# zengyf131/gswt_renderer

Measured on AMD Instinct MI355X. Metric: frames/sec @1920x1080, 32x32 Wang-tile grid, higher is better.
Workload: dtype f32

## Files before the change

gswt_renderer_amd/_lib.py:

```python
from __future__ import annotations

import ctypes as C
import os

_HERE = os.path.dirname(os.path.abspath(__file__))
LIB_PATH = os.environ.get("GSWT_HIP_LIB") or os.path.join(_HERE, "lib", "libgswt_hip.so")

GSWT_OK = 0
GSWT_ERR_BAD_ARG = -1
GSWT_ERR_CAPACITY = -2
GSWT_ERR_HIP = -3
GSWT_ERR_STATE = -4
GSWT_ERR_RCCL = -6
GSWT_COMM_ID_BYTES = 128
GSWT_ORDER_REFERENCE = 0
GSWT_ORDER_DEPTH = 1
GSWT_OPT_NO_LOD_PREFILTER = 1
GSWT_OPT_DEBUG_VARYINGS = 2
GSWT_OPT_SEGMENT = 3
GSWT_DEFAULT_SEGMENT = 1536
GSWT_OPT_DEBUG_FLAGS = 4
GSWT_OPT_TIMING = 5
GSWT_OPT_PAIR_CAP = 6
GSWT_OPT_NO_MERGE_REUSE = 7
GSWT_OPT_DEFER_SWAP = 8
GSWT_OPT_GRAPH = 9
GSWT_OPT_STRICT_VS = 10
GSWT_OPT_DEPTH_PASSES = 12
GSWT_OPT_COMPOSITE = 13
GSWT_OPT_DEPTH_SORT = 14
GSWT_OPT_NO_CHUNK_CULL = 15
GSWT_OPT_ITEM_ORDER = 16
GSWT_SCENE_TEX = 0
GSWT_SCENE_RAW_DEPTH = 1
GSWT_SCENE_RAW_TABLES = 2
GSWT_SCENE_STATIC_LIST = 3
GSWT_SCENE_STATIC_BOXES = 4
GSWT_SCENE_LISTS = 5
GSWT_SCENE_BOUNDS = 6
GSWT_SHARD_ROWS = 0
GSWT_SHARD_COLUMNS = 1
GSWT_OUT_RGBA32F = 0
GSWT_OUT_RGBA8_UNORM = 1
GSWT_OUT_BGRA8_UNORM = 2
GSWT_VIDEO_NV12 = 16
GSWT_VIDEO_I420 = 17
GSWT_PROXY_SRC_RGBA8 = 0
GSWT_PROXY_SRC_RGBA16 = 1


class CameraUniforms(C.Structure):
    _fields_ = [("projection", C.c_float * 16), ("view", C.c_float * 16), ("focal", C.c_float * 2),
                ("viewport", C.c_float * 2), ("htan_fov", C.c_float * 4), ("cam_pos", C.c_float * 4)]


class SceneUniforms(C.Structure):
    _fields_ = [("splat_scale", C.c_float), ("tile_width", C.c_float), ("use_clip", C.c_uint32),
                ("clip_height", C.c_float), ("surface_type", C.c_uint32), ("sphere_radius", C.c_float),
                ("point_cloud_radius", C.c_float), ("transition_width_ratio", C.c_float),
                ("num_lod", C.c_uint32), ("draw_mode", C.c_uint32), ("map_half_wh", C.c_uint32 * 2),
                ("center_coord", C.c_int32 * 2), ("_pad0", C.c_uint32 * 2),
                ("transition_dist_vec", C.c_float * 16), ("height_map_scale", C.c_float * 4),
                ("scene_scale", C.c_float * 4)]


class TileUniforms(C.Structure):
    _fields_ = [("single_draw", C.c_uint32), ("map_index", C.c_uint32), ("single_lod_id", C.c_int32),
                ("valid_lod_id", C.c_int32), ("changing", C.c_uint32), ("changing_to_lower", C.c_int32),
                ("_pad0", C.c_uint32 * 2), ("tile_id", C.c_uint32 * 4), ("offset", C.c_float * 4),
                ("map_coord", C.c_uint32 * 4)]


# ... 179 lines not shown
```

gswt_renderer_amd/csrc/gswt_api.hip:

```cpp
#include "../../include/gswt_hip.h"
#include "gswt_device.h"

#include <dlfcn.h>

#include <algorithm>
#include <cstdarg>
#include <cstdio>
#include <cstring>
#include <string>
#include <unordered_map>
#include <utility>
#include <vector>

using namespace gswt;

namespace {

template <typename T>
struct DevBuf {
    T* p = nullptr;
    size_t cap = 0;
    DevBuf() = default;
    DevBuf(DevBuf&& o) noexcept : p(std::exchange(o.p, nullptr)), cap(std::exchange(o.cap, 0)) {}
    DevBuf& operator=(DevBuf&& o) noexcept { std::swap(p, o.p); std::swap(cap, o.cap); return *this; }
// ... 774 lines not shown
    c->static_n = arena_n; c->boxes_n = boxes_n;
    c->raw_cnt.assign(counts, counts + n_lt);
    c->raw_merge_offset = moff;
    c->raw_off.assign(n_lt * nv, 0);
    for (size_t i = 0; i < n_lt; i++) for (size_t v = 0; v < nv; v++) c->raw_off[i * nv + v] = (uint32_t)(nv * moff[i] + v * counts[i]);
    c->n_lod = n_lod; c->n_tile = n_tile; c->n_view = n_view;
    c->scene_ready = true;
    return GSWT_OK;
} GSWT_CATCH("gswt_upload_scene_rows")

int gswt_debug_read_scene(gswt_ctx* c, int what, void* out, size_t cap_bytes, size_t* n_bytes)
try {
    if (!c || !n_bytes) return GSWT_ERR_BAD_ARG;
    if (!c->scene_ready) return fail(c, GSWT_ERR_STATE, "gswt_debug_read_scene before a scene upload");
    const void* dev = nullptr;
    const void* hostp = nullptr;
    size_t bytes = 0;
    std::vector<uint32_t> tmp;
    switch (what) {
    case GSWT_SCENE_TEX: dev = c->tex.p; bytes = c->n_splats * 32; break;
    case GSWT_SCENE_RAW_DEPTH: {
        size_t total = 0;
        for (uint32_t k : c->raw_cnt) total += (size_t)k * c->n_view;
        dev = c->raw_depth.p; bytes = total * 4; break;
    }
    case GSWT_SCENE_RAW_TABLES:
        tmp = c->raw_off;
        tmp.insert(tmp.end(), c->raw_cnt.begin(), c->raw_cnt.end());
        tmp.insert(tmp.end(), c->raw_merge_offset.begin(), c->raw_merge_offset.end());
        hostp = tmp.data(); bytes = tmp.size() * 4; break;
    case GSWT_SCENE_STATIC_LIST: dev = c->static_list.p; bytes = c->static_n * 4; break;
    case GSWT_SCENE_STATIC_BOXES: dev = c->static_boxes.p; bytes = c->boxes_n * 24; break;
    case GSWT_SCENE_LISTS: hostp = c->lists.data(); bytes = c->lists.size() * sizeof(ListRef); break;
    case GSWT_SCENE_BOUNDS: {
        tmp.resize(7);
        memcpy(tmp.data(), c->loc_lo, 12); memcpy(tmp.data() + 3, c->loc_hi, 12); memcpy(tmp.data() + 6, &c->loc_max_trace, 4);
        hostp = tmp.data(); bytes = 28; break;
    }
    default: return fail(c, GSWT_ERR_BAD_ARG, "gswt_debug_read_scene: unknown item %d", what);
    }
    *n_bytes = bytes;
    if (!out) return GSWT_OK;
    if (cap_bytes < bytes) return fail(c, GSWT_ERR_CAPACITY, "gswt_debug_read_scene: buffer holds %zu bytes, need %zu", cap_bytes, bytes);
    if (hostp) { memcpy(out, hostp, bytes); return GSWT_OK; }
    hipSetDevice(c->device);
    HIP_TRY(c, sync_all(c));
    if (bytes) HIP_TRY(c, hipMemcpy(out, dev, bytes, hipMemcpyDeviceToHost));
    return GSWT_OK;
} GSWT_CATCH("gswt_debug_read_scene")

int gswt_configure(gswt_ctx* c, const float* height_map, int hm_w, int hm_h)
try {
    if (!c) return GSWT_ERR_BAD_ARG;
    hipSetDevice(c->device);
    HIP_TRY(c, collect_pending(c));
    if (!height_map || hm_w <= 0 || hm_h <= 0) { c->hm_w = c->hm_h = 0; return GSWT_OK; }
    HIP_TRY(c, c->hmap.ensure((size_t)hm_w * hm_h + 2));
    HIP_TRY(c, hipMemcpy(c->hmap.p, height_map, (size_t)hm_w * hm_h * 4, hipMemcpyHostToDevice));
    HIP_TRY(c, hipMemset(c->hmap.p + (size_t)hm_w * hm_h, 0, 8));
    {
        float mn = height_map[0], mx = height_map[0], du = 0.f, dv = 0.f;
        bool finite = true;
        for (int y = 0; y < hm_h; y++)
            for (int x = 0; x < hm_w; x++) {
                const float h = height_map[(size_t)y * hm_w + x];
                const float hr = height_map[(size_t)y * hm_w + (x + 1 == hm_w ? 0 : x + 1)], hd = height_map[(size_t)(y + 1 == hm_h ? 0 : y + 1) * hm_w + x];
// ... 309 lines not shown
        total += len;
    }
    if (total >= 0xFFFFFFFFull) return fail(c, GSWT_ERR_CAPACITY, "gswt_set_draws_merge_groups: merged lists exceed 2^32 entries");
    for (int i = 0; i < n_draws; i++)
        if (draws[i].merged) {
            const uint32_t g = draws[i].merged_group;
            if ((int)g >= n_groups || draws[i].merged_offset != desc[g].base || draws[i].merged_count != desc[g].len)
                return fail(c, GSWT_ERR_BAD_ARG, "gswt_set_draws_merge_groups: draw %d does not match group %u (offset %u/%u count %u/%u)", i, g,
                            draws[i].merged_offset, (int)g < n_groups ? desc[g].base : 0u, draws[i].merged_count, (int)g < n_groups ? desc[g].len : 0u);
        }
    int rc = set_draws_impl(c, draws, n_draws, nullptr, nullptr, nullptr, (size_t)total, true);
    if (rc != GSWT_OK) return rc;
    MergeSources msrc;
    for (int k = 0; k < kMergeSources; k++) { msrc.list[k] = nullptr; msrc.map[k] = nullptr; }
    D.src_mask = 0;
    for (int k : sources) {
        if (!c->sets[k].g_valid) return fail(c, GSWT_ERR_STATE, "gswt_set_draws_merge_groups: a source set lost its lists");
        msrc.list[k] = c->sets[k].merged_list.p; msrc.map[k] = c->sets[k].merged_map.p;
    }
    for (size_t q = 0; q < n_jobs; q++) D.src_mask |= 1u << jobs[q].src_set;
    D.g_desc.swap(desc);
    D.g_members.assign(members, members + n_members);
    D.g_valid = false;
    c->stat_groups_built += n_build; c->stat_groups_reused += n_jobs;
    hipStream_t s = c->set_stream;
    uint2* const h_cblocks = D.hp<uint2>(D.off_cblocks);
    uint2* const h_blocks = D.hp<uint2>(D.off_blocks);
    size_t n_cb = 0, n_blocks = 0;
    for (size_t q = 0; q < n_jobs; q++)
        for (uint32_t off = 0; off < jobs[q].len; off += 1024u) h_cblocks[n_cb++] = make_uint2((uint32_t)q, off);
    for (size_t q = 0; q < n_segs; q++)
        for (uint32_t off = 0; off < segs[q].len; off += 1024u) h_blocks[n_blocks++] = make_uint2((uint32_t)q, off);
    const uint32_t n_total = (uint32_t)build_total;
    memset(D.hp<uint8_t>(D.off_n64), 0, 64);
    *D.hp<unsigned long long>(D.off_n64) = n_total;
    HIP_TRY(c, hipMemcpyAsync(D.d_blob.p, D.h_blob.p, D.blob_bytes, hipMemcpyHostToDevice, s));
    launch_chunk_tabs(s, D.draws.p, D.xcd_first.p, D.n_draws, D.chunk_tab.p, D.chunk_tab_xcd.p, D.per_xcd, D.longest);
    if (n_jobs)
        launch_merge_copy(s, D.dp<MergeCopy>(D.off_jobs), D.dp<uint2>(D.off_cblocks), (uint32_t)n_cb, D.dp<uint2>(D.off_remap), msrc,
                          D.merged_list.p, D.merged_map.p);
    if (n_build) {
        int gbits = 1;
        while ((1u << gbits) < n_build) gbits++;
        const size_t radix_words = radix_ws_words(n_total, 16 + gbits);
        HIP_TRY(c, c->mg_ws.ensure_roomy(4 * (size_t)n_total + radix_words + 16));
        uint32_t* w = c->mg_ws.p;
        uint32_t* radix = w + 4 * (size_t)n_total;
        HIP_TRY(c, hipMemsetAsync(radix, 0, (radix_words + 16) * 4, s));
        launch_merge_build(s, D.dp<MergeSeg>(D.off_segs), (uint32_t)n_segs, D.dp<uint2>(D.off_blocks), (uint32_t)n_blocks, D.dp<MergeGroup>(D.off_groups),
                           (uint32_t)n_build, c->raw_depth.p, n_total, D.dp<unsigned long long>(D.off_n64), w, w + n_total, w + 2 * (size_t)n_total,
                           w + 3 * (size_t)n_total, radix, gbits, D.merged_list.p, D.merged_map.p);
    }
    HIP_TRY(c, hipGetLastError());
    HIP_TRY(c, hipEventRecord(D.ev_up, s));
    D.ev_up_pending = true; D.built = false;
    D.g_valid = true;
    publish_set(c, target);
    c->draws_ready = true;
    return GSWT_OK;
} GSWT_CATCH("gswt_set_draws_merge_groups")

int gswt_debug_read_merged(gswt_ctx* c, uint32_t* packed_list, uint32_t* map_id, size_t capacity, size_t* n)
try {
    if (!c || !n) return GSWT_ERR_BAD_ARG;
    const DrawSet& D = c->sets[c->cur_set];
    *n = D.n_merged;
    if (!packed_list || !map_id) return GSWT_OK;
    if (capacity < D.n_merged) return fail(c, GSWT_ERR_CAPACITY, "buffer holds %zu entries, need %zu", capacity, D.n_merged);
    hipSetDevice(c->device);
    HIP_TRY(c, sync_all(c));
    if (D.n_merged) {
        HIP_TRY(c, hipMemcpy(packed_list, D.merged_list.p, D.n_merged * 4, hipMemcpyDeviceToHost));
        HIP_TRY(c, hipMemcpy(map_id, D.merged_map.p, D.n_merged * 4, hipMemcpyDeviceToHost));
    }
    return GSWT_OK;
} GSWT_CATCH("gswt_debug_read_merged")

int gswt_shard_rows_padded(int height, int shard_count)
try {
    int tiles_y = (height + kTile - 1) / kTile;
    int sc = shard_count <= 1 ? 1 : shard_count;
// ... 1079 lines not shown
```

gswt_renderer_amd/csrc/gswt_device.h:

```cpp
#pragma once
#include <hip/hip_runtime.h>
#include <hip/hip_ext.h>
#include <hip/hip_fp16.h>
#include <stdint.h>
#include <string.h>
#include <type_traits>

namespace gswt {

constexpr int kTile = 16;
constexpr int kChunk = 256;
constexpr uint32_t kLodShift = 28;
constexpr uint32_t kIdxMask = (1u << kLodShift) - 1u;
constexpr int kOutF32 = 0, kOutRGBA8 = 1, kOutBGRA8 = 2;
constexpr int kOutNV12 = 16, kOutI420 = 17;
constexpr bool out_is_video(int out_format) { return out_format == kOutNV12 || out_format == kOutI420; }
inline size_t out_image_bytes(int out_format, int rows, int out_w)
{
    if (rows < 0 || out_w < 0) return 0;
    const size_t px = (size_t)rows * (size_t)out_w;
    if (out_format == kOutF32) return px * 16u;
    if (out_format == kOutRGBA8 || out_format == kOutBGRA8) return px * 4u;
    if (out_is_video(out_format)) return ((rows | out_w) & 1) ? 0 : px + px / 2u;
    return 0;
// ... 222 lines not shown
    uint2* partials_pick;
    hipEvent_t ev_pick_begin, ev_pick_end;
    uint32_t n_zero_head, n_zero_ranges, n_zero_depth;
};

void launch_chunk_tabs(hipStream_t s, const DrawDev* draws, const uint32_t* xcd_first, uint32_t n_draws, uint2* chunk_tab, uint2* chunk_tab_xcd,
                       const uint64_t per_xcd[8], uint64_t longest);
void launch_merge_build(hipStream_t s, const MergeSeg* segs, uint32_t n_segs, const uint2* blocks, uint32_t n_blocks, MergeGroup* groups, uint32_t n_groups,
                        const int32_t* raw, uint32_t n_total, const unsigned long long* n_total_dev, uint32_t* ka, uint32_t* va,
                        uint32_t* kb, uint32_t* vb, uint32_t* radix_ws, int group_bits, uint32_t* merged_list, uint32_t* merged_map);
int launch_scene_sort(hipStream_t s, const MergeSeg* segs, const uint2* blocks, uint32_t n_blocks, MergeGroup* groups, const int32_t* raw,
                      uint32_t n_total, const unsigned long long* n_total_dev, uint32_t* ka, uint32_t* va, uint32_t* kb, uint32_t* vb,
                      uint32_t* radix_ws, int group_bits);
void launch_scene_tex(hipStream_t s, const uint4* rows, uint32_t n, uint4* tex, int32_t* bounds);
void launch_scene_raw(hipStream_t s, const uint4* rows, uint32_t n, const uint32_t* moff, const uint32_t* cnt, uint32_t n_lt, const SceneViews& vps,
                      int32_t* raw);
void launch_scene_scatter(hipStream_t s, const MergeSeg* segs, uint32_t n_segs, const MergeGroup* groups, const uint32_t* sorted_keys,
                          const uint32_t* sorted_vals, uint32_t n_total, uint32_t* arena, uint32_t arena_n);
void launch_scene_self(hipStream_t s, const SceneList* lists, uint32_t n_lists, uint32_t lists_per_lod, uint32_t* arena);
void launch_scene_boxes(hipStream_t s, const SceneList* lists, uint32_t n_lists, uint32_t n_boxes, const uint32_t* arena, const uint4* tex,
                        uint32_t n_splats, float* boxes);
void launch_merge_copy(hipStream_t s, const MergeCopy* jobs, const uint2* blocks, uint32_t n_blocks, const uint2* remap, const MergeSources& src,
                       uint32_t* new_list, uint32_t* new_map);

void launch_cull(hipStream_t s, const Frame& f, const FrameBufs& b, bool chunk_cull);
void launch_project(hipStream_t s, const Frame& f, const FrameBufs& b, uint32_t n_launch, bool debug, bool strict);
void launch_emit(hipStream_t s, const Frame& f, const FrameBufs& b, uint32_t* keys, uint32_t* dkeys, uint32_t* krange, uint32_t n_launch);
void launch_composite(hipStream_t s, const Frame& f, const FrameBufs& b, const uint32_t* vals, int out_rows, int variant, const uint32_t* krange,
                      uint32_t depth_passes, bool report_max, bool heavy_first, hipEvent_t ev_begin, hipEvent_t ev_end, int out_format);
void launch_totals(hipStream_t s, uint32_t* super_sums, uint32_t n_super, unsigned long long* counters, uint32_t pair_cap);

size_t radix_ws_words(uint32_t n_cap, int key_bits);
size_t radix_ws_zero_words(uint32_t n_cap, int key_bits);
int launch_sort(hipStream_t s, uint32_t* keys_a, uint32_t* vals_a, uint32_t* keys_b, uint32_t* vals_b, uint32_t n_cap,
                const unsigned long long* n_ptr, int key_bits, uint32_t* ws, uint2* ranges = nullptr, const uint32_t* krange = nullptr,
                uint32_t* aux_a = nullptr, uint32_t* aux_b = nullptr);

void launch_tile_depth_sort(hipStream_t s, const uint2* ranges, uint32_t* vals, uint32_t* dkeys, uint32_t* vals_scratch, uint32_t* dkeys_scratch, int n_tiles,
                            uint32_t* long_list, unsigned long long* counters);
inline size_t tile_depth_list_words(size_t n_tiles) { return n_tiles + 1; }
uint32_t tile_depth_sort_cap();

void launch_unshard(hipStream_t s, const void* gathered, void* out, int width, int height, int shard_count, int rows_padded, int band_px,
                    int out_format);
void launch_skybox(hipStream_t s, const float* view16, float p00, float p11, int width, int height, int face_size, int equirect,
                   const float4* faces, float4* out);
void launch_skybox_bake(hipStream_t s, const SkyBakeArgs& a, const float4* equi, float4* faces);
void launch_proxy(hipStream_t s, const ProxyArgs& a, const float* hm, const float4* tex, float4* rgba, float* depth);
void launch_proxy_mip(hipStream_t s, const ProxyMipArgs& a, const uint8_t* src, int2* ranges, float* wv, float* wh, float4* tmp,
                      float4* part, float4* dst);
void launch_fill_f32(hipStream_t s, float* p, size_t n, float v);

}
```

gswt_renderer_amd/csrc/gswt_kernels.hip:

```cpp
#include "gswt_device.h"

namespace gswt {

__device__ __forceinline__ unsigned long long ballot64(bool p) { return __builtin_amdgcn_ballot_w64(p); }
__device__ __forceinline__ uint32_t lanes_below(unsigned long long m)
{
    return __builtin_amdgcn_mbcnt_hi((uint32_t)(m >> 32), __builtin_amdgcn_mbcnt_lo((uint32_t)m, 0u));
}

template <int CTRL, int ROW_MASK>
__device__ __forceinline__ uint32_t dpp_or_zero(uint32_t x)
{
    return (uint32_t)__builtin_amdgcn_update_dpp(0, (int)x, CTRL, ROW_MASK, 0xF, true);
}
__device__ __forceinline__ uint32_t wave_incl_scan(uint32_t v, uint32_t lane)
{
    (void)lane;
    v += dpp_or_zero<0x111, 0xF>(v);
    v += dpp_or_zero<0x112, 0xF>(v);
    v += dpp_or_zero<0x114, 0xF>(v);
    v += dpp_or_zero<0x118, 0xF>(v);
    v += dpp_or_zero<0x142, 0xA>(v);
    v += dpp_or_zero<0x143, 0xC>(v);
    return v;
// ... 164 lines not shown
        if (f.draw_mode == 3u) L = d.single_lod_id >= 0 ? (uint32_t)d.single_lod_id : lod_id;
        float cx = 0.0f, cy = 1.0f;
        if (L < 3u) cx = (3.0f - (float)L) / 3.0f;
        else cy = (6.0f - (float)L) / 3.0f;
        cr = 0.5f; cg = cx; cb = cy;
    } else if (f.draw_mode == 4u) {
        const uint32_t v = d.tile_view;
        float cx = 0.0f, cy = 0.0f;
        if (v < 4u) cx = (4.0f - (float)v) / 4.0f;
        if (v >= 4u) cy = (8.0f - (float)v) / 4.0f;
        if (v >= 8u) { cx = 1.0f; cy = 1.0f; }
        cr = 0.5f; cg = cx; cb = cy;
    }
}

__device__ __forceinline__ void tile_xy(const Frame& f, uint32_t tile, int& tx, int& ty)
{
    uint32_t q;
    if (f.tiles_x_magic != 0u && tile < 65536u) q = __umulhi(tile, f.tiles_x_magic);
    else q = tile / (uint32_t)f.tiles_x;
    tx = (int)(tile - q * (uint32_t)f.tiles_x); ty = (int)q;
}

__device__ __forceinline__ int owned_rows(int ty0, int ty1, int index, int count)
{
    if (count <= 1) return ty1 - ty0 + 1;
    int first = ty0 + ((index - ty0 % count) + count) % count;
    if (first > ty1) return 0;
    return (ty1 - first) / count + 1;
}

struct XcdLens { uint32_t len[8]; uint32_t longest; };
__global__ __launch_bounds__(256) void k_chunk_tabs(const DrawDev* __restrict__ draws, const uint32_t* __restrict__ xcd_first, uint32_t n_draws,
                                                    uint2* __restrict__ chunk_tab, uint2* __restrict__ chunk_tab_xcd, const XcdLens xl)
{
    const uint32_t d = blockIdx.x;
    if (d >= n_draws) {
        const uint32_t x = d - n_draws;
        for (uint32_t k = xl.len[x & 7u] + threadIdx.x; k < xl.longest; k += 256u) chunk_tab_xcd[(size_t)k * 8u + x] = make_uint2(0xFFFFFFFFu, 0xFFFFFFFFu);
        return;
    }
    const uint32_t nch = (draws[d].count + (uint32_t)kChunk - 1u) / (uint32_t)kChunk;
    const uint32_t c0 = draws[d].slot_base / (uint32_t)kChunk, x0 = xcd_first[d];
    for (uint32_t k = threadIdx.x; k < nch; k += 256u) {
        const uint2 e = make_uint2(d, k * (uint32_t)kChunk);
        chunk_tab[c0 + k] = e;
        chunk_tab_xcd[(size_t)(x0 + k) * 8u + (draws[d].xcd & 7u)] = e;
    }
}

__device__ __forceinline__ bool sphere_cell_box(const Frame& f, float bidx, float bidy, const float lo[3], const float hi[3], float blo[3], float bhi[3])
{
    const float xmax = ((float)f.map_half_wh[0] * 2.0f) * f.tile_width;
    const float block_w = xmax / 5.0f;
    const float ox = (float)(f.center_coord[0] - (int32_t)f.map_half_wh[0]) * f.tile_width + bidx * block_w;
    const float oy = (float)(f.center_coord[1] - (int32_t)f.map_half_wh[1]) * f.tile_width + bidy * block_w;
    const float bx0 = lo[0] - ox, bx1 = hi[0] - ox, by0 = lo[1] - oy, by1 = hi[1] - oy;
    if (!(block_w > 0.0f && bx0 >= 0.0f && bx1 <= block_w && by0 >= 0.0f && by1 <= block_w)) return false;
    constexpr int n = 3;
    const float R = fabsf(f.sphere_radius);
    const float zmax = fmaxf(fabsf(lo[2]), fabsf(hi[2]));
    const float rho = (R * 2.5f * ((bx1 - bx0) + (by1 - by0)) / (2.0f * (float)n * block_w) + zmax) * 1.02f + 1e-4f * R;
    if (!(rho == rho)) return false;
    for (int k = 0; k < 3; k++) { blo[k] = 3.402823466e+38f; bhi[k] = -3.402823466e+38f; }
    for (int j = 0; j < n; j++)
        for (int i = 0; i < n; i++) {
            float p[3];
            sphere_point(block_w, bidx, bidy, bx0 + (bx1 - bx0) * (((float)i + 0.5f) / (float)n), by0 + (by1 - by0) * (((float)j + 0.5f) / (float)n), p);
            for (int k = 0; k < 3; k++) { blo[k] = fminf(blo[k], p[k] * f.sphere_radius - rho); bhi[k] = fmaxf(bhi[k], p[k] * f.sphere_radius + rho); }
        }
    return blo[0] == blo[0] && bhi[0] == bhi[0] && blo[1] == blo[1] && bhi[1] == bhi[1] && blo[2] == blo[2] && bhi[2] == bhi[2];
}

__device__ __forceinline__ bool band_misses(const Frame& f, const float lo[3], const float hi[3], float bidx, float bidy)
{
    float blo[3], bhi[3];
    for (int k = 0; k < 3; k++) {
        const float a = lo[k] * f.scene_scale[k], b = hi[k] * f.scene_scale[k];
        blo[k] = fminf(a, b); bhi[k] = fmaxf(a, b);
    }
    if (f.surface_type == 1u) {
// ... 1004 lines not shown
        }
    }
    __syncthreads();
    GSWT_TR(4, GSWT_NOW())
    const uint32_t n_blk = min((uint32_t)kSortBlock, n - blk0);
#pragma unroll
    for (int k = 0; k < kSortItems; k++) {
        const uint32_t i = (uint32_t)k * kSortThreads + threadIdx.x;
        if (i < n_blk) {
            const uint2 kv = s_kv[i];
            const uint32_t gp = s_g[((kv.x - kmin) >> shift) & mask] + i;
            vals_out[gp] = kv.y;
            if (AUX == 2) aux_out[gp] = s_aux[AUX == 2 ? i : 0u];
            if (AUX == 1) aux_out[gp] = aux_in[blk0 + s_src[AUX == 1 ? i : 0u]];
            if (!ranges) keys_out[gp] = kv.x;
            else {
                const uint32_t kp = s_kv[i == 0u ? 0u : i - 1u].x, kn = s_kv[min(i + 1u, n_blk - 1u)].x;
                if (i == 0u || kp != kv.x) atomicMax(&ranges[kv.x].x, ~gp);
                if (i == n_blk - 1u || kn != kv.x) atomicMax(&ranges[kv.x].y, gp + 1u);
            }
        }
    }
    GSWT_TR(5, GSWT_NOW())
}

__device__ __forceinline__ uint32_t mg_find_seg(const MergeSeg* __restrict__ segs, uint32_t n_segs, uint32_t e)
{
    uint32_t lo = 0, hi = n_segs;
    while (hi - lo > 1u) { const uint32_t mid = (lo + hi) >> 1; if (segs[mid].start <= e) lo = mid; else hi = mid; }
    return lo;
}

__global__ __launch_bounds__(256) void k_mg_minmax(const MergeSeg* __restrict__ segs, const uint2* __restrict__ blocks, const int32_t* __restrict__ raw,
                                                   MergeGroup* __restrict__ groups)
{
    __shared__ int32_t s_mn[4], s_mx[4];
    const uint2 b = blocks[blockIdx.x];
    const MergeSeg sg = segs[b.x];
    int32_t mn = 2147483647, mx = -2147483647 - 1;
#pragma unroll
    for (uint32_t k = 0; k < 4u; k++) {
        const uint32_t i = b.y + k * 256u + threadIdx.x;
        const int32_t d = raw[sg.src + min(i, sg.len - 1u)];
        mn = min(mn, d); mx = max(mx, d);
    }
    for (int off = 32; off > 0; off >>= 1) { mn = min(mn, __shfl_down(mn, off, 64)); mx = max(mx, __shfl_down(mx, off, 64)); }
    if ((threadIdx.x & 63u) == 0) { s_mn[threadIdx.x >> 6] = mn; s_mx[threadIdx.x >> 6] = mx; }
    __syncthreads();
    if (threadIdx.x == 0) {
        atomicMin(&groups[sg.group].mn, min(min(s_mn[0], s_mn[1]), min(s_mn[2], s_mn[3])));
        atomicMax(&groups[sg.group].mx, max(max(s_mx[0], s_mx[1]), max(s_mx[2], s_mx[3])));
    }
}

__global__ __launch_bounds__(256) void k_mg_keys(const MergeSeg* __restrict__ segs, const uint2* __restrict__ blocks, const int32_t* __restrict__ raw,
                                                 const MergeGroup* __restrict__ groups, uint32_t* __restrict__ keys, uint32_t* __restrict__ vals)
{
    const uint2 b = blocks[blockIdx.x];
    const MergeSeg sg = segs[b.x];
    const MergeGroup g = groups[sg.group];
    const float depth_inv = 65535.0f / (float)(int32_t)((uint32_t)g.mx - (uint32_t)g.mn);
#pragma unroll
    for (uint32_t k = 0; k < 4u; k++) {
        const uint32_t i = b.y + k * 256u + threadIdx.x;
        if (i >= sg.len) break;
        const int32_t d = raw[sg.src + i];
        const float v = floorf((float)(int32_t)((uint32_t)d - (uint32_t)g.mn) * depth_inv);
        int32_t bk;
        if (v != v) bk = 0;
// ... 1000 lines not shown
        const int shard = x / band_px;
        src = ((size_t)shard * height + y) * band_px + (x - shard * band_px);
    } else {
        int ty = y >> 4;
        int shard = ty % shard_count, tyl = ty / shard_count;
        src = ((size_t)shard * rows_padded + (size_t)tyl * kTile + (y & 15)) * width + x;
    }
    out[(size_t)y * width + x] = gathered[src];
}

template <typename P, int TILE>
__global__ void k_unshard_plane(const P* __restrict__ gathered, P* __restrict__ out, int width, int height,
                                int shard_count, int rows_padded, int band_px, size_t stride)
{
    const int x = blockIdx.x * blockDim.x + threadIdx.x;
    const int y = blockIdx.y;
    if (x >= width || y >= height) return;
    size_t src;
    if (band_px > 0) {
        const int shard = x / band_px;
        src = (size_t)shard * stride + (size_t)y * band_px + (x - shard * band_px);
    } else {
        const int ty = y / TILE;
        const int shard = ty % shard_count, tyl = ty / shard_count;
        src = (size_t)shard * stride + ((size_t)tyl * TILE + (y % TILE)) * width + x;
    }
    out[(size_t)y * width + x] = gathered[src];
}

void launch_chunk_tabs(hipStream_t s, const DrawDev* draws, const uint32_t* xcd_first, uint32_t n_draws, uint2* chunk_tab, uint2* chunk_tab_xcd,
                       const uint64_t per_xcd[8], uint64_t longest)
{
    XcdLens xl;
    for (int x = 0; x < 8; x++) xl.len[x] = (uint32_t)per_xcd[x];
    xl.longest = (uint32_t)longest;
    if (n_draws) hipLaunchKernelGGL(k_chunk_tabs, dim3(n_draws + 8u), dim3(256), 0, s, draws, xcd_first, n_draws, chunk_tab, chunk_tab_xcd, xl);
}

GraphRec*& graph_recorder()
{
    static thread_local GraphRec* rec = nullptr;
    return rec;
}

bool kernel_events_enabled()
{
    static const bool on = !(getenv("GSWT_KERNEL_EVENTS") && atoi(getenv("GSWT_KERNEL_EVENTS")) == 0);
    return on;
}

void launch_cull(hipStream_t s, const Frame& f, const FrameBufs& b, bool chunk_cull)
{
    uint32_t grid = (b.n_chunks + 255u) / 256u;
    if (grid < 32) grid = 32;
    GSWT_LAUNCH(k_cull, dim3(grid), dim3(256), s, f, b.draws, b.draw_culled, b.cell_culled, b.n_cells, reinterpret_cast<uint32_t*>(b.counters), b.n_zero_head,
                reinterpret_cast<uint32_t*>(b.ranges), b.n_zero_ranges, b.block_sums, b.n_chunks, b.radix_depth, b.n_zero_depth,
                b.chunk_tab, b.n_chunks, b.boxes, chunk_cull && b.boxes ? 1u : 0u, b.live_cnt, b.live_tab, b.live_cid);
}

void launch_project(hipStream_t s, const Frame& f, const FrameBufs& b, uint32_t n_launch, bool debug, bool strict)
{
    if (b.n_chunks == 0) return;
    const uint32_t n_super = b.n_chunks / 256u + 1u;
    const bool full = f.surface_type == 2u || f.draw_mode != 0u;
#define GSWT_LAUNCH_PROJECT_S(D, F, S)                                                                                         \
    GSWT_LAUNCH((k_project<D, F, S>), dim3(n_launch), dim3(256), s, f, b.draws, b.chunk_tab_xcd, b.static_list, b.merged_list,   \
                b.merged_map, b.tex, b.hmap, b.draw_culled, b.cell_culled, b.live_cnt, b.live_tab, b.rects, b.recs, b.depths, b.block_sums, \
                b.super_sums, n_super, b.dbg, b.col_f)
#define GSWT_LAUNCH_PROJECT(D, F) do { if (strict) GSWT_LAUNCH_PROJECT_S(D, F, true); else GSWT_LAUNCH_PROJECT_S(D, F, false); } while (0)
// ... 7 lines not shown
}

void launch_emit(hipStream_t s, const Frame& f, const FrameBufs& b, uint32_t* keys, uint32_t* dkeys, uint32_t* krange, uint32_t n_launch)
{
    const uint32_t n_chunks = b.n_chunks, pair_cap = b.pair_cap;
    if (n_chunks == 0) return;
    const uint32_t n_super = n_chunks / 256u + 1u;
    const uint32_t* const excl = b.super_sums + 2u * kSuperStride * n_super;
    const float* const no_f = nullptr; uint32_t* const no_u = nullptr;
    const uint32_t* const cnt2 = n_launch ? b.live_cnt + 8u * kSuperStride : nullptr;
    const uint32_t* const cid = n_launch ? b.live_cid : nullptr;
    const dim3 grid(n_launch ? ((n_launch / 8u + kEmitGroup - 1u) / kEmitGroup) * 8u : (n_chunks + kEmitGroup - 1u) / kEmitGroup);
#define GSWT_LAUNCH_EMIT(D, L)                                                                                                 \
    GSWT_LAUNCH((k_emit<D, L>), grid, dim3(256), s, f, b.rects, b.block_sums, excl, n_chunks, pair_cap, b.counters, keys, b.vals_a, \
                D ? b.depths : no_f, D ? dkeys : no_u, D ? krange : no_u, cnt2, cid)
    if (n_launch) { if (dkeys) GSWT_LAUNCH_EMIT(true, true); else GSWT_LAUNCH_EMIT(false, true); }
    else if (dkeys) GSWT_LAUNCH_EMIT(true, false);
    else GSWT_LAUNCH_EMIT(false, false);
#undef GSWT_LAUNCH_EMIT
}

size_t radix_ws_words(uint32_t n_cap, int key_bits)
{
    const uint32_t nblk = (n_cap + kSortBlock - 1) / kSortBlock, nsup = (nblk >> kSupShift) + 1;
    const int passes = (key_bits + 7) / 8;
    return (size_t)passes * ((size_t)256 * nblk + (size_t)256 * nsup + 256);
}
size_t radix_ws_zero_words(uint32_t n_cap, int key_bits)
{
    const uint32_t nblk = (n_cap + kSortBlock - 1) / kSortBlock, nsup = (nblk >> kSupShift) + 1;
    const int passes = (key_bits + 7) / 8;
    return (size_t)passes * ((size_t)256 * nsup + 256);
}

int launch_sort(hipStream_t s, uint32_t* keys_a, uint32_t* vals_a, uint32_t* keys_b, uint32_t* vals_b, uint32_t n_cap,
                const unsigned long long* n_ptr, int key_bits, uint32_t* ws, uint2* ranges, const uint32_t* krange, uint32_t* aux_a, uint32_t* aux_b)
{
    if (n_cap == 0) return 0;
    const uint32_t nblk = (n_cap + kSortBlock - 1) / kSortBlock, nsup = (nblk >> kSupShift) + 1;
    const int threads = n_cap <= kSortWideMax ? 512 : 256;
    int cur = 0;
    const int passes = (key_bits + 7) / 8;
    uint32_t* hist_rows = ws + (size_t)passes * ((size_t)256 * nsup + 256);
    for (int shift = 0; shift < key_bits; shift += 8) {
        uint32_t nbits = (uint32_t)((key_bits - shift) < 8 ? (key_bits - shift) : 8);
        uint32_t mask = (1u << nbits) - 1u;
        uint32_t* gsup = ws; uint32_t* gtot = gsup + (size_t)256 * nsup;
        ws = gtot + 256;
        uint32_t* ghist = hist_rows;
        hist_rows += (size_t)256 * nblk;
        uint32_t* ki = cur ? keys_b : keys_a; uint32_t* vi = cur ? vals_b : vals_a;
        uint32_t* ko = cur ? keys_a : keys_b; uint32_t* vo = cur ? vals_a : vals_b;
        const uint32_t* xi = cur ? aux_b : aux_a; uint32_t* xo = cur ? aux_a : aux_b;
#define GSWT_SORT_PASS(T)                                                                                                        \
        GSWT_LAUNCH(k_radix_hist<T>, dim3(nblk), dim3(T), s, ki, n_ptr, n_cap, (uint32_t)shift, mask, nbits, ghist, gsup, gtot, nblk, nsup, krange); \
        if (nsup > kSupDirect) GSWT_LAUNCH(k_radix_supscan, dim3(64), dim3(256), s, gsup, gtot, nsup);                          \
        if (aux_a && n_cap > (12u << 20)) GSWT_LAUNCH((k_radix_scatter<T, 2>), dim3(nblk), dim3(T), s, ki, vi, ko, vo, n_ptr, n_cap, (uint32_t)shift, mask, nbits, \
                           ghist, gsup, gtot, nblk, nsup, shift + 8 >= key_bits ? ranges : (uint2*)nullptr, krange, xi, xo);                  \
        else if (aux_a) GSWT_LAUNCH((k_radix_scatter<T, 1>), dim3(nblk), dim3(T), s, ki, vi, ko, vo, n_ptr, n_cap, (uint32_t)shift, mask, nbits,    \
                           ghist, gsup, gtot, nblk, nsup, shift + 8 >= key_bits ? ranges : (uint2*)nullptr, krange, xi, xo);                  \
        else GSWT_LAUNCH((k_radix_scatter<T, 0>), dim3(nblk), dim3(T), s, ki, vi, ko, vo, n_ptr, n_cap, (uint32_t)shift, mask, nbits,    \
                           ghist, gsup, gtot, nblk, nsup, shift + 8 >= key_bits ? ranges : (uint2*)nullptr, krange, xi, xo)
        if (threads == 512) { GSWT_SORT_PASS(512); }
        else { GSWT_SORT_PASS(256); }
#undef GSWT_SORT_PASS
        cur ^= 1;
    }
    return cur;
}

void launch_merge_build(hipStream_t s, const MergeSeg* segs, uint32_t n_segs, const uint2* blocks, uint32_t n_blocks, MergeGroup* groups, uint32_t n_groups,
                        const int32_t* raw, uint32_t n_total, const unsigned long long* n_total_dev, uint32_t* ka, uint32_t* va,
                        uint32_t* kb, uint32_t* vb, uint32_t* radix_ws, int group_bits, uint32_t* merged_list, uint32_t* merged_map)
{
    if (n_total == 0 || n_groups == 0 || n_blocks == 0) return;
    hipLaunchKernelGGL(k_mg_minmax, dim3(n_blocks), dim3(256), 0, s, segs, blocks, raw, groups);
    hipLaunchKernelGGL(k_mg_keys, dim3(n_blocks), dim3(256), 0, s, segs, blocks, raw, groups, ka, va);
    const int where = launch_sort(s, ka, va, kb, vb, n_total, n_total_dev, 16 + group_bits, radix_ws);
    hipLaunchKernelGGL(k_mg_final, dim3((n_total + 255) / 256), dim3(256), 0, s, segs, n_segs, groups, where ? kb : ka, where ? vb : va,
                       n_total, merged_list, merged_map);
}

int launch_scene_sort(hipStream_t s, const MergeSeg* segs, const uint2* blocks, uint32_t n_blocks, MergeGroup* groups, const int32_t* raw,
                      uint32_t n_total, const unsigned long long* n_total_dev, uint32_t* ka, uint32_t* va, uint32_t* kb, uint32_t* vb,
                      uint32_t* radix_ws, int group_bits)
{
    if (n_total == 0 || n_blocks == 0) return 0;
    hipLaunchKernelGGL(k_mg_minmax, dim3(n_blocks), dim3(256), 0, s, segs, blocks, raw, groups);
    hipLaunchKernelGGL(k_mg_keys, dim3(n_blocks), dim3(256), 0, s, segs, blocks, raw, groups, ka, va);
    return launch_sort(s, ka, va, kb, vb, n_total, n_total_dev, 16 + group_bits, radix_ws);
}

void launch_merge_copy(hipStream_t s, const MergeCopy* jobs, const uint2* blocks, uint32_t n_blocks, const uint2* remap, const MergeSources& src,
                       uint32_t* new_list, uint32_t* new_map)
{
    if (n_blocks) hipLaunchKernelGGL(k_mg_copy, dim3(n_blocks), dim3(256), 0, s, jobs, blocks, remap, src, new_list, new_map);
}

void launch_tile_depth_sort(hipStream_t s, const uint2* ranges, uint32_t* vals, uint32_t* dkeys, uint32_t* vals_scratch, uint32_t* dkeys_scratch, int n_tiles,
                            uint32_t* long_list, unsigned long long* counters)
{
    if (n_tiles <= 0) return;
    const uint32_t nt = (uint32_t)n_tiles;
    GSWT_LAUNCH((k_tile_depth_sort<64, 8, false>), dim3(nt), dim3(64), s, ranges, vals, dkeys, nt, long_list, counters, 0u, 0u, vals_scratch, dkeys_scratch);
    GSWT_LAUNCH((k_tile_depth_sort<256, 16, false>), dim3(nt), dim3(256), s, ranges, vals, dkeys, nt, long_list, counters, 512u, 1u, vals_scratch, dkeys_scratch);
    GSWT_LAUNCH((k_tile_depth_sort<1024, 16, true>), dim3(kTileSortLongGrid), dim3(1024), s, ranges, vals, dkeys, nt, long_list, counters, 4096u, 0u,
                vals_scratch, dkeys_scratch);
}
uint32_t tile_depth_sort_cap() { return kTileSortCap; }

template <typename Fn>
static void with_composite_edc(const Frame& f, Fn&& fn)
{
    const bool early = f.t_eps > 0.0f, depth = f.has_depth != 0, colf = f.draw_mode != 0u;
    using T = std::true_type;
    using F = std::false_type;
    if (colf) { if (depth) fn(F{}, T{}, T{}); else fn(F{}, F{}, T{}); }
    else if (early && depth) fn(T{}, T{}, F{});
    else if (early) fn(T{}, F{}, F{});
    else if (depth) fn(F{}, T{}, F{});
    else fn(F{}, F{}, F{});
// ... 108 lines not shown
```

include/gswt_hip.h:

```cpp
#ifndef GSWT_HIP_H
#define GSWT_HIP_H

#include <stddef.h>
#include <stdint.h>

#ifdef __cplusplus
extern "C" {
#endif

#define GSWT_API __attribute__((visibility("default")))

typedef struct gswt_ctx gswt_ctx;

enum {
    GSWT_OK = 0,
    GSWT_ERR_BAD_ARG = -1,
    GSWT_ERR_CAPACITY = -2,
    GSWT_ERR_HIP = -3,
    GSWT_ERR_STATE = -4,
    GSWT_ERR_RCCL = -6
};

enum { GSWT_ORDER_REFERENCE = 0, GSWT_ORDER_DEPTH = 1 };

// ... 116 lines not shown
       GSWT_OPT_NO_CHUNK_CULL = 15 ,
       GSWT_OPT_ITEM_ORDER = 16  };
GSWT_API int gswt_set_option(gswt_ctx *ctx, int key, int value);

GSWT_API int gswt_upload_scene(gswt_ctx *ctx, const uint32_t *tex_data, size_t n_splats,
                               const gswt_base_list *lists, int n_lod, int n_tile, int n_view);

GSWT_API int gswt_configure(gswt_ctx *ctx, const float *height_map, int hm_w, int hm_h);

GSWT_API int gswt_set_draws(gswt_ctx *ctx, const gswt_draw *draws, int n_draws,
                            const uint32_t *merged_gs_index, const uint32_t *merged_map_id,
                            const uint32_t *merged_lod_id, size_t n_merged);

typedef struct {
    uint32_t view_id;
    uint32_t first_member;
    uint32_t n_members;
    uint32_t _pad;
} gswt_merge_group;
typedef struct {
    uint32_t map_index;
    uint32_t lod, tile;
    int32_t other_lod;
} gswt_merge_member;
GSWT_API int gswt_upload_raw_depth(gswt_ctx *ctx, const int32_t *const *raw_depth ,
                                   const uint32_t *counts ,
                                   const uint32_t *merge_offset );
GSWT_API int gswt_set_draws_merge_groups(gswt_ctx *ctx, const gswt_draw *draws, int n_draws,
                                         const gswt_merge_group *groups, int n_groups,
                                         const gswt_merge_member *members, int n_members);
GSWT_API int gswt_upload_scene_rows(gswt_ctx *ctx, const uint8_t *const *rows32, const uint32_t *counts, int n_lod, int n_tile,
                                    const float *presort_vp, int n_view);
enum { GSWT_SCENE_TEX = 0, GSWT_SCENE_RAW_DEPTH = 1, GSWT_SCENE_RAW_TABLES = 2, GSWT_SCENE_STATIC_LIST = 3, GSWT_SCENE_STATIC_BOXES = 4,
       GSWT_SCENE_LISTS = 5, GSWT_SCENE_BOUNDS = 6 };
GSWT_API int gswt_debug_read_scene(gswt_ctx *ctx, int what, void *out, size_t cap_bytes, size_t *n_bytes);
GSWT_API int gswt_debug_read_merged(gswt_ctx *ctx, uint32_t *packed_list, uint32_t *map_id, size_t capacity, size_t *n);

GSWT_API int gswt_render(gswt_ctx *ctx, const gswt_camera_uniforms *camera,
                         const gswt_scene_uniforms *scene, const gswt_render_config *cfg,
                         int width, int height,
                         const float *bg_rgba, const float *bg_depth, int bg_on_device,
                         float *out_rgba, int out_on_device);

GSWT_API int gswt_render_async(gswt_ctx *ctx, const gswt_camera_uniforms *camera,
                               const gswt_scene_uniforms *scene, const gswt_render_config *cfg,
                               int width, int height, const float *bg_rgba_dev, const float *bg_depth_dev,
                               float *out_rgba_dev, int *ticket);
GSWT_API int gswt_frame_slots(void);

GSWT_API int gswt_render_depth(gswt_ctx *ctx, const gswt_camera_uniforms *camera,
                               const gswt_scene_uniforms *scene, const gswt_render_config *cfg,
                               int width, int height,
                               const float *bg_rgba, const float *bg_depth, int bg_on_device,
                               float *out_rgba, float *out_depth, int out_on_device);
GSWT_API int gswt_render_async_depth(gswt_ctx *ctx, const gswt_camera_uniforms *camera,
                                     const gswt_scene_uniforms *scene, const gswt_render_config *cfg,
                                     int width, int height, const float *bg_rgba_dev, const float *bg_depth_dev,
                                     float *out_rgba_dev, float *out_depth_dev, int *ticket);

typedef struct {
    uint32_t map_index;
    uint32_t entry;
    float depth;
    float weight;
} gswt_pick;
GSWT_API int gswt_render_pick(gswt_ctx *ctx, const gswt_camera_uniforms *camera,
                              const gswt_scene_uniforms *scene, const gswt_render_config *cfg,
// ... 177 lines not shown
```

rust/src/gswt_hip_sys.rs:

```rust
#![allow(non_camel_case_types, dead_code)]
use std::os::raw::{c_char, c_int, c_uint, c_void};

pub const GSWT_OK: c_int = 0;
pub const GSWT_ERR_BAD_ARG: c_int = -1;
pub const GSWT_ERR_CAPACITY: c_int = -2;
pub const GSWT_ERR_HIP: c_int = -3;
pub const GSWT_ERR_STATE: c_int = -4;
pub const GSWT_ERR_RCCL: c_int = -6;
pub const GSWT_ORDER_REFERENCE: c_int = 0;
pub const GSWT_ORDER_DEPTH: c_int = 1;
pub const GSWT_SHARD_ROWS: c_int = 0;
pub const GSWT_SHARD_COLUMNS: c_int = 1;
pub const GSWT_OUT_RGBA32F: c_int = 0;
pub const GSWT_OUT_RGBA8_UNORM: c_int = 1;
pub const GSWT_OUT_BGRA8_UNORM: c_int = 2;
pub const GSWT_VIDEO_NV12: c_int = 16;
pub const GSWT_VIDEO_I420: c_int = 17;
pub const GSWT_OPT_NO_LOD_PREFILTER: c_int = 1;
pub const GSWT_OPT_DEBUG_VARYINGS: c_int = 2;
pub const GSWT_OPT_SEGMENT: c_int = 3;
pub const GSWT_OPT_DEBUG_FLAGS: c_int = 4;
pub const GSWT_OPT_TIMING: c_int = 5;
pub const GSWT_OPT_PAIR_CAP: c_int = 6;
pub const GSWT_OPT_NO_MERGE_REUSE: c_int = 7;
pub const GSWT_OPT_DEFER_SWAP: c_int = 8;
pub const GSWT_OPT_GRAPH: c_int = 9;
pub const GSWT_OPT_STRICT_VS: c_int = 10;
pub const GSWT_OPT_DEPTH_PASSES: c_int = 12;
pub const GSWT_OPT_COMPOSITE: c_int = 13;
pub const GSWT_OPT_DEPTH_SORT: c_int = 14;
pub const GSWT_OPT_NO_CHUNK_CULL: c_int = 15;
pub const GSWT_OPT_ITEM_ORDER: c_int = 16;
pub const GSWT_SCENE_TEX: c_int = 0;
pub const GSWT_SCENE_RAW_DEPTH: c_int = 1;
pub const GSWT_SCENE_RAW_TABLES: c_int = 2;
pub const GSWT_SCENE_STATIC_LIST: c_int = 3;
pub const GSWT_SCENE_STATIC_BOXES: c_int = 4;
pub const GSWT_SCENE_LISTS: c_int = 5;
pub const GSWT_SCENE_BOUNDS: c_int = 6;
pub const GSWT_PROXY_SRC_RGBA8: c_int = 0;
pub const GSWT_PROXY_SRC_RGBA16: c_int = 1;
pub const GSWT_COMM_ID_BYTES: c_int = 128;

#[repr(C)] pub struct GswtCtx { _private: [u8; 0] }
#[repr(C)] pub struct GswtWorker { _private: [u8; 0] }

#[repr(C)] #[derive(Clone, Copy)]
pub struct GswtCameraUniforms {
    pub projection: [f32; 16],
    pub view: [f32; 16],
    pub focal: [f32; 2],
    pub viewport: [f32; 2],
    pub htan_fov: [f32; 4],
    pub cam_pos: [f32; 4],
}

#[repr(C)] #[derive(Clone, Copy)]
pub struct GswtSceneUniforms {
    pub splat_scale: f32,
    pub tile_width: f32,
    pub use_clip: u32,
    pub clip_height: f32,
    pub surface_type: u32,
    pub sphere_radius: f32,
    pub point_cloud_radius: f32,
    pub transition_width_ratio: f32,
    pub num_lod: u32,
    pub draw_mode: u32,
    pub map_half_wh: [u32; 2],
    pub center_coord: [i32; 2],
    pub _pad0: [u32; 2],
    pub transition_dist_vec: [f32; 16],
// ... 487 lines not shown
```

Baseline: 5613.

## Flatten chunk-table build to per-chunk threads and fold radix zeroing into minmax

Rewrites k_chunk_tabs from one block per draw looping over chunks to one thread per chunk slot. Each thread binary-searches the draws by slot_base, and the XCD padding fill is spread across threads. Also removes the separate hipMemsetAsync of the radix workspace by zeroing it inside k_mg_minmax, which saves a stream operation per merge build. It adds debug readback items for the chunk tables and an env-gated log line. The fold assumes k_mg_minmax always runs before the sort consumes the workspace, and the binary search assumes draws are sorted by slot_base.

```diff
diff --git a/gswt_renderer_amd/_lib.py b/gswt_renderer_amd/_lib.py
--- a/gswt_renderer_amd/_lib.py
+++ b/gswt_renderer_amd/_lib.py
@@ -38,6 +38,9 @@
 GSWT_SCENE_STATIC_BOXES = 4
 GSWT_SCENE_LISTS = 5
 GSWT_SCENE_BOUNDS = 6
+GSWT_SCENE_CHUNK_TAB = 7
+GSWT_SCENE_CHUNK_TAB_XCD = 8
+GSWT_SCENE_DRAW_CHUNKS = 9
 GSWT_SHARD_ROWS = 0
 GSWT_SHARD_COLUMNS = 1
 GSWT_OUT_RGBA32F = 0
diff --git a/gswt_renderer_amd/csrc/gswt_api.hip b/gswt_renderer_amd/csrc/gswt_api.hip
--- a/gswt_renderer_amd/csrc/gswt_api.hip
+++ b/gswt_renderer_amd/csrc/gswt_api.hip
@@ -830,6 +830,29 @@
     case GSWT_SCENE_STATIC_LIST: dev = c->static_list.p; bytes = c->static_n * 4; break;
     case GSWT_SCENE_STATIC_BOXES: dev = c->static_boxes.p; bytes = c->boxes_n * 24; break;
     case GSWT_SCENE_LISTS: hostp = c->lists.data(); bytes = c->lists.size() * sizeof(ListRef); break;
+    case GSWT_SCENE_CHUNK_TAB: case GSWT_SCENE_CHUNK_TAB_XCD: {
+        const DrawSet& D = c->sets[c->cur_set];
+        if (!c->draws_ready) return fail(c, GSWT_ERR_STATE, "gswt_debug_read_scene: no draw list yet");
+        if (what == GSWT_SCENE_CHUNK_TAB) { dev = D.chunk_tab.p; bytes = (size_t)D.n_chunks * 8; }
+        else { dev = D.chunk_tab_xcd.p; bytes = (size_t)D.n_launch * 8; }
+        break;
+    }
+    case GSWT_SCENE_DRAW_CHUNKS: {
+        const DrawSet& D = c->sets[c->cur_set];
+        if (!c->draws_ready) return fail(c, GSWT_ERR_STATE, "gswt_debug_read_scene: no draw list yet");
+        bytes = (size_t)D.n_draws * 16;
+        if (out && cap_bytes >= bytes && D.n_draws) {
+            std::vector<DrawDev> dd(D.n_draws);
+            std::vector<uint32_t> xf(D.n_draws);
+            hipSetDevice(c->device);
+            HIP_TRY(c, sync_all(c));
+            HIP_TRY(c, hipMemcpy(dd.data(), D.draws.p, dd.size() * sizeof(DrawDev), hipMemcpyDeviceToHost));
+            HIP_TRY(c, hipMemcpy(xf.data(), D.xcd_first.p, xf.size() * 4, hipMemcpyDeviceToHost));
+            tmp.resize((size_t)D.n_draws * 4);
+            for (uint32_t i = 0; i < D.n_draws; i++) { tmp[4 * i] = dd[i].count; tmp[4 * i + 1] = dd[i].slot_base; tmp[4 * i + 2] = dd[i].xcd; tmp[4 * i + 3] = xf[i]; }
+        } else tmp.resize(1);
+        hostp = tmp.data(); break;
+    }
     case GSWT_SCENE_BOUNDS: {
         tmp.resize(7);
         memcpy(tmp.data(), c->loc_lo, 12); memcpy(tmp.data() + 3, c->loc_hi, 12); memcpy(tmp.data() + 6, &c->loc_max_trace, 4);
@@ -1205,6 +1228,16 @@
     for (size_t q = 0; q < n_segs; q++)
         for (uint32_t off = 0; off < segs[q].len; off += 1024u) h_blocks[n_blocks++] = make_uint2((uint32_t)q, off);
     const uint32_t n_total = (uint32_t)build_total;
+    {
+        static const bool log_events = getenv("GSWT_LOG_SORT_EVENTS") != nullptr;
+        if (log_events) {
+            int gb = 1;
+            while ((1u << gb) < n_build) gb++;
+            fprintf(stderr, "gswt sort event: n_draws %d n_chunks %u n_total %u n_build %zu n_jobs %zu n_blocks %zu n_cblocks %zu nblk %u passes %d\n", n_draws,
+                    D.n_chunks, n_total, n_build, n_jobs, n_blocks, n_cb, n_build ? (n_total + sort_block_items() - 1) / sort_block_items() : 0u,
+                    n_build ? (16 + gb + 7) / 8 : 0);
+        }
+    }
     memset(D.hp<uint8_t>(D.off_n64), 0, 64);
     *D.hp<unsigned long long>(D.off_n64) = n_total;
     HIP_TRY(c, hipMemcpyAsync(D.d_blob.p, D.h_blob.p, D.blob_bytes, hipMemcpyHostToDevice, s));
@@ -1219,7 +1252,6 @@
         HIP_TRY(c, c->mg_ws.ensure_roomy(4 * (size_t)n_total + radix_words + 16));
         uint32_t* w = c->mg_ws.p;
         uint32_t* radix = w + 4 * (size_t)n_total;
-        HIP_TRY(c, hipMemsetAsync(radix, 0, (radix_words + 16) * 4, s));
         launch_merge_build(s, D.dp<MergeSeg>(D.off_segs), (uint32_t)n_segs, D.dp<uint2>(D.off_blocks), (uint32_t)n_blocks, D.dp<MergeGroup>(D.off_groups),
                            (uint32_t)n_build, c->raw_depth.p, n_total, D.dp<unsigned long long>(D.off_n64), w, w + n_total, w + 2 * (size_t)n_total,
                            w + 3 * (size_t)n_total, radix, gbits, D.merged_list.p, D.merged_map.p);
diff --git a/gswt_renderer_amd/csrc/gswt_device.h b/gswt_renderer_amd/csrc/gswt_device.h
--- a/gswt_renderer_amd/csrc/gswt_device.h
+++ b/gswt_renderer_amd/csrc/gswt_device.h
@@ -278,6 +278,7 @@
 
 size_t radix_ws_words(uint32_t n_cap, int key_bits);
 size_t radix_ws_zero_words(uint32_t n_cap, int key_bits);
+uint32_t sort_block_items();
 int launch_sort(hipStream_t s, uint32_t* keys_a, uint32_t* vals_a, uint32_t* keys_b, uint32_t* vals_b, uint32_t n_cap,
                 const unsigned long long* n_ptr, int key_bits, uint32_t* ws, uint2* ranges = nullptr, const uint32_t* krange = nullptr,
                 uint32_t* aux_a = nullptr, uint32_t* aux_b = nullptr);
diff --git a/gswt_renderer_amd/csrc/gswt_kernels.hip b/gswt_renderer_amd/csrc/gswt_kernels.hip
--- a/gswt_renderer_amd/csrc/gswt_kernels.hip
+++ b/gswt_renderer_amd/csrc/gswt_kernels.hip
@@ -220,21 +220,27 @@
 
 struct XcdLens { uint32_t len[8]; uint32_t longest; };
 __global__ __launch_bounds__(256) void k_chunk_tabs(const DrawDev* __restrict__ draws, const uint32_t* __restrict__ xcd_first, uint32_t n_draws,
-                                                    uint2* __restrict__ chunk_tab, uint2* __restrict__ chunk_tab_xcd, const XcdLens xl)
-{
-    const uint32_t d = blockIdx.x;
-    if (d >= n_draws) {
-        const uint32_t x = d - n_draws;
-        for (uint32_t k = xl.len[x & 7u] + threadIdx.x; k < xl.longest; k += 256u) chunk_tab_xcd[(size_t)k * 8u + x] = make_uint2(0xFFFFFFFFu, 0xFFFFFFFFu);
+                                                    uint32_t n_chunks, uint2* __restrict__ chunk_tab, uint2* __restrict__ chunk_tab_xcd, const XcdLens xl)
+{
+    const uint32_t t = blockIdx.x * 256u + threadIdx.x;
+    if (t >= xl.longest * 8u) return;
+    if (t >= n_chunks) {
+        uint32_t p = t - n_chunks;
+        for (uint32_t x = 0; x < 8u; x++) {
+            const uint32_t gap = xl.longest - xl.len[x];
+            if (p < gap) { chunk_tab_xcd[(size_t)(xl.len[x] + p) * 8u + x] = make_uint2(0xFFFFFFFFu, 0xFFFFFFFFu); return; }
+            p -= gap;
+        }
         return;
     }
-    const uint32_t nch = (draws[d].count + (uint32_t)kChunk - 1u) / (uint32_t)kChunk;
-    const uint32_t c0 = draws[d].slot_base / (uint32_t)kChunk, x0 = xcd_first[d];
-    for (uint32_t k = threadIdx.x; k < nch; k += 256u) {
-        const uint2 e = make_uint2(d, k * (uint32_t)kChunk);
-        chunk_tab[c0 + k] = e;
-        chunk_tab_xcd[(size_t)(x0 + k) * 8u + (draws[d].xcd & 7u)] = e;
-    }
+    const uint32_t slot = t * (uint32_t)kChunk;
+    uint32_t lo = 0, hi = n_draws - 1u;
+    while (lo < hi) { const uint32_t mid = (lo + hi) >> 1; if (draws[mid].slot_base <= slot) hi = mid; else lo = mid + 1u; }
+    const uint32_t d = lo;
+    const uint32_t k = t - draws[d].slot_base / (uint32_t)kChunk;
+    const uint2 e = make_uint2(d, k * (uint32_t)kChunk);
+    chunk_tab[t] = e;
+    chunk_tab_xcd[(size_t)(xcd_first[d] + k) * 8u + (draws[d].xcd & 7u)] = e;
 }
 
 __device__ __forceinline__ bool sphere_cell_box(const Frame& f, float bidx, float bidy, const float lo[3], const float hi[3], float blo[3], float bhi[3])
@@ -1305,9 +1311,11 @@
 }
 
 __global__ __launch_bounds__(256) void k_mg_minmax(const MergeSeg* __restrict__ segs, const uint2* __restrict__ blocks, const int32_t* __restrict__ raw,
-                                                   MergeGroup* __restrict__ groups)
+                                                   MergeGroup* __restrict__ groups, uint32_t* __restrict__ zero_ws, uint32_t n_zero, size_t zero_tail)
 {
     __shared__ int32_t s_mn[4], s_mx[4];
+    if (zero_ws)
+        for (uint32_t i = blockIdx.x * 256u + threadIdx.x; i < n_zero + 16u; i += gridDim.x * 256u) zero_ws[i < n_zero ? (size_t)i : zero_tail + (i - n_zero)] = 0u;
     const uint2 b = blocks[blockIdx.x];
     const MergeSeg sg = segs[b.x];
     int32_t mn = 2147483647, mx = -2147483647 - 1;
@@ -2374,9 +2382,12 @@
                        const uint64_t per_xcd[8], uint64_t longest)
 {
     XcdLens xl;
-    for (int x = 0; x < 8; x++) xl.len[x] = (uint32_t)per_xcd[x];
+    uint64_t n_chunks = 0;
+    for (int x = 0; x < 8; x++) { xl.len[x] = (uint32_t)per_xcd[x]; n_chunks += per_xcd[x]; }
     xl.longest = (uint32_t)longest;
-    if (n_draws) hipLaunchKernelGGL(k_chunk_tabs, dim3(n_draws + 8u), dim3(256), 0, s, draws, xcd_first, n_draws, chunk_tab, chunk_tab_xcd, xl);
+    const uint32_t n_pos = (uint32_t)(longest * 8u);
+    if (n_draws && n_pos)
+        hipLaunchKernelGGL(k_chunk_tabs, dim3((n_pos + 255u) / 256u), dim3(256), 0, s, draws, xcd_first, n_draws, (uint32_t)n_chunks, chunk_tab, chunk_tab_xcd, xl);
 }
 
 GraphRec*& graph_recorder()
@@ -2450,6 +2461,8 @@
     const int passes = (key_bits + 7) / 8;
     return (size_t)passes * ((size_t)256 * nsup + 256);
 }
+
+uint32_t sort_block_items() { return (uint32_t)kSortBlock; }
 
 int launch_sort(hipStream_t s, uint32_t* keys_a, uint32_t* vals_a, uint32_t* keys_b, uint32_t* vals_b, uint32_t n_cap,
                 const unsigned long long* n_ptr, int key_bits, uint32_t* ws, uint2* ranges, const uint32_t* krange, uint32_t* aux_a, uint32_t* aux_b)
@@ -2492,7 +2505,8 @@
                         uint32_t* kb, uint32_t* vb, uint32_t* radix_ws, int group_bits, uint32_t* merged_list, uint32_t* merged_map)
 {
     if (n_total == 0 || n_groups == 0 || n_blocks == 0) return;
-    hipLaunchKernelGGL(k_mg_minmax, dim3(n_blocks), dim3(256), 0, s, segs, blocks, raw, groups);
+    hipLaunchKernelGGL(k_mg_minmax, dim3(n_blocks), dim3(256), 0, s, segs, blocks, raw, groups, radix_ws,
+                       (uint32_t)radix_ws_zero_words(n_total, 16 + group_bits), radix_ws_words(n_total, 16 + group_bits));
     hipLaunchKernelGGL(k_mg_keys, dim3(n_blocks), dim3(256), 0, s, segs, blocks, raw, groups, ka, va);
     const int where = launch_sort(s, ka, va, kb, vb, n_total, n_total_dev, 16 + group_bits, radix_ws);
     hipLaunchKernelGGL(k_mg_final, dim3((n_total + 255) / 256), dim3(256), 0, s, segs, n_segs, groups, where ? kb : ka, where ? vb : va,
@@ -2504,7 +2518,7 @@
                       uint32_t* radix_ws, int group_bits)
 {
     if (n_total == 0 || n_blocks == 0) return 0;
-    hipLaunchKernelGGL(k_mg_minmax, dim3(n_blocks), dim3(256), 0, s, segs, blocks, raw, groups);
+    hipLaunchKernelGGL(k_mg_minmax, dim3(n_blocks), dim3(256), 0, s, segs, blocks, raw, groups, (uint32_t*)nullptr, 0u, (size_t)0);
     hipLaunchKernelGGL(k_mg_keys, dim3(n_blocks), dim3(256), 0, s, segs, blocks, raw, groups, ka, va);
     return launch_sort(s, ka, va, kb, vb, n_total, n_total_dev, 16 + group_bits, radix_ws);
 }
diff --git a/include/gswt_hip.h b/include/gswt_hip.h
--- a/include/gswt_hip.h
+++ b/include/gswt_hip.h
@@ -172,7 +172,7 @@
 GSWT_API int gswt_upload_scene_rows(gswt_ctx *ctx, const uint8_t *const *rows32, const uint32_t *counts, int n_lod, int n_tile,
                                     const float *presort_vp, int n_view);
 enum { GSWT_SCENE_TEX = 0, GSWT_SCENE_RAW_DEPTH = 1, GSWT_SCENE_RAW_TABLES = 2, GSWT_SCENE_STATIC_LIST = 3, GSWT_SCENE_STATIC_BOXES = 4,
-       GSWT_SCENE_LISTS = 5, GSWT_SCENE_BOUNDS = 6 };
+       GSWT_SCENE_LISTS = 5, GSWT_SCENE_BOUNDS = 6, GSWT_SCENE_CHUNK_TAB = 7, GSWT_SCENE_CHUNK_TAB_XCD = 8, GSWT_SCENE_DRAW_CHUNKS = 9 };
 GSWT_API int gswt_debug_read_scene(gswt_ctx *ctx, int what, void *out, size_t cap_bytes, size_t *n_bytes);
 GSWT_API int gswt_debug_read_merged(gswt_ctx *ctx, uint32_t *packed_list, uint32_t *map_id, size_t capacity, size_t *n);
 
diff --git a/rust/src/gswt_hip_sys.rs b/rust/src/gswt_hip_sys.rs
--- a/rust/src/gswt_hip_sys.rs
+++ b/rust/src/gswt_hip_sys.rs
@@ -38,6 +38,9 @@
 pub const GSWT_SCENE_STATIC_BOXES: c_int = 4;
 pub const GSWT_SCENE_LISTS: c_int = 5;
 pub const GSWT_SCENE_BOUNDS: c_int = 6;
+pub const GSWT_SCENE_CHUNK_TAB: c_int = 7;
+pub const GSWT_SCENE_CHUNK_TAB_XCD: c_int = 8;
+pub const GSWT_SCENE_DRAW_CHUNKS: c_int = 9;
 pub const GSWT_PROXY_SRC_RGBA8: c_int = 0;
 pub const GSWT_PROXY_SRC_RGBA16: c_int = 1;
 pub const GSWT_COMM_ID_BYTES: c_int = 128;
```

Result: no change. 5625, median of 4 (+0.2%).
